# Niravaana/HIP-BVH-Construction

Hardware: AMD Instinct MI355X
Metric: bvh_build_throughput (higher is better)
Workload: dtype f32+u32

## Files before the change

### hip-bvh-construction_amd/csrc/api.hip

```cpp
#include <hip/hip_runtime.h>
#include <new>
#include <cstring>
#include <cstdlib>
#include "bvh_mi355x.h"
#include <mutex>
#include "common.hpp"
#include "kernels.hpp"

#include <vector>
#include <string>
#include <map>

using namespace bvh;

namespace bvh { thread_local KernelRecorder* g_recorder = nullptr; }

struct EventRecorder : KernelRecorder {
    struct Rec { const char* name; hipEvent_t ev; };
    std::vector<Rec> recs; size_t used = 0;
    std::string only;
    bool open = false;
    void mark(hipStream_t s, const char* name) override {
        if (!only.empty()) {
            const bool match = name && only == name;
// ... 11 lines not shown
struct bvh_ctx {
    int device = 0;
    hipStream_t stream = nullptr;
    bool own_stream = false;
    bool profiling = false;
    bool kernel_profiling = false;
    uint32_t sample_every = 1, build_counter = 0;
    EventRecorder recorder;
    uint32_t cap = 0;
    char* arena = nullptr;
    size_t arena_bytes = 0;
    void* tris = nullptr;
    uint32_t tris_cap = 0;
    bvh_aabb* boxes = nullptr;
    float* scene = nullptr;
    u32 *keys = nullptr, *skeys = nullptr, *svals = nullptr;
    SortScratch sort{};
    bvh2_node* nodes = nullptr;
    bvh_primref* leaves = nullptr;
    u64* slots = nullptr;
    u32* parent = nullptr;
    u32* flags = nullptr;
    HplocScratch hploc{};
    PlocScratch ploc{};
    u32* small = nullptr;
    u64* overlap_sums = nullptr;
    size_t lbvh_queue_capacity = 0;
    bool scratch_dirty = false;
    hipEvent_t ev[8] = {};
    int scene_slot = 0;
    bool scene_ready = false;
    uint32_t ploc_last_n = 0, ploc_last_iters = 0;
    u32* h_pinned = nullptr;
    u32* d_pinned = nullptr;
    float last_collapse_ms = 0.f;
    uint32_t collapse_last_n = 0, collapse_last_levels = 0;
    uint64_t collapse_last_key = 0;
    uint32_t collapse_last_len[COLLAPSE_MAX_BATCH] = {0};
    int collapse_len_batch = 0;
    int64_t options[4] = {0, 0, 0, 0};
    uint64_t tree_serial = 1, plan_serial = 0;
    uint32_t plan_n = 0, plan_root = 0;
    u32* subset_words = nullptr;
    uint32_t subset_cap = 0;
    bool subset_dirty = false;
    uint64_t map_serial = 0;
// ... 63 lines not shown
    __atomic_thread_fence(__ATOMIC_RELEASE);
}
static int read_back(bvh_ctx* c, const u32* d_a, u32 na, const u32* d_b, u32 nb, u32* pairs);

inline size_t align_up(size_t v, size_t a = 256) { return (v + a - 1) / a * a; }

struct Carver {
    char* base; size_t off = 0;
    template <typename T> T* take(size_t count) { T* p = base ? reinterpret_cast<T*>(base + off) : nullptr; off += align_up(count * sizeof(T)); return p; }
};

void carve(bvh_ctx* c, char* base, uint32_t cap, size_t* total) {
    Carver k{base};
    const size_t n = cap;
    c->boxes = k.take<bvh_aabb>(n);
    c->scene = k.take<float>(16);
    c->keys = reinterpret_cast<u32*>(k.take<u64>(n)); c->skeys = reinterpret_cast<u32*>(k.take<u64>(n)); c->svals = k.take<u32>(n);
    c->sort.pairs0 = k.take<uint4>(n); c->sort.pairs1 = k.take<uint4>(n);
    c->sort.hist = k.take<u32>(SORT_HIST_COPIES * SORT_HIST_STRIDE);
    c->sort.status = k.take<u32>(sort_status_bytes(cap) / sizeof(u32));
    c->sort.counters = k.take<u32>(SORT_MAX_PASSES);
    c->nodes = k.take<bvh2_node>(2 * n);
    c->leaves = k.take<bvh_primref>(n);
    c->slots = k.take<u64>(n);
    c->parent = k.take<u32>(2 * n);
    c->flags = k.take<u32>(n);
    c->hploc.recs = k.take<bvh2_node>(n);
    c->hploc.dep = k.take<u64>(n);
    c->hploc.queue_capacity = hploc_queue_capacity(cap);
    c->hploc.queue_pc = k.take<u32>(c->hploc.queue_capacity);
    c->hploc.queue_rng = k.take<u64>(c->hploc.queue_capacity);
// ... 11 lines not shown
}
inline u32* overflow_words(const bvh_ctx* c) { return c->small + 58; }
inline u64* total_word(const bvh_ctx* c) { return reinterpret_cast<u64*>(c->small + 60); }
inline u32* total_pairs(const bvh_ctx* c) { return c->h_pinned + 8; }

int ensure_capacity(bvh_ctx* c, uint32_t n) {
    if (n <= c->cap) return 0;
    HIP_TRY(hipStreamSynchronize(c->stream));
    if (c->arena) { HIP_TRY(hipFree(c->arena)); c->arena = nullptr; c->cap = 0; }
    size_t total = 0;
    carve(c, nullptr, n, &total);
    char* p = nullptr;
    HIP_TRY(hipMalloc(&p, total));
    c->arena = p; c->arena_bytes = total; c->cap = n;
    ++c->tree_serial;
    c->scene_ready = false; c->scene_slot = 0;
    carve(c, p, n, &total);
    HIP_TRY(hipMemsetAsync(c->hploc.dep, 0, (size_t)n * sizeof(u64), c->stream));
    HIP_TRY(hipMemsetAsync(c->flags, 0xFF, (size_t)n * sizeof(u32), c->stream));
    return 0;
}

int begin_emit(bvh_ctx* c) {
    if (c->scratch_dirty) {
        HIP_TRY(hipMemsetAsync(c->hploc.dep, 0, (size_t)c->cap * sizeof(u64), c->stream));
        HIP_TRY(hipMemsetAsync(c->flags, 0xFF, (size_t)c->cap * sizeof(u32), c->stream));
    }
    c->scratch_dirty = true;
    return 0;
}
int end_emit(bvh_ctx* c) {
// ... 64 lines not shown
            return 0;
        }
        first += batch; batch = 16;
    }
    return BVH_E_INTERNAL;
}

int stage_extents_valid(const bvh_build_input* in) {
    switch (in->tri_format) {
        case BVH_TRI_PADDED64: return in->d_tris ? 0 : BVH_E_INVALID_ARG;
        case BVH_TRI_PACKED36: return (in->d_tris && !((uintptr_t)in->d_tris & 15u)) ? 0 : BVH_E_INVALID_ARG;
        case BVH_TRI_INDEXED:  return (in->d_vertices && in->d_indices && in->n_vertices) ? 0 : BVH_E_INVALID_ARG;
        default: return BVH_E_INVALID_ARG;
    }
}
int stage_extents_fmt(hipStream_t s, const bvh_build_input* in, uint32_t n, void* d_boxes, void* d_scene, bool reset_scene = true, const PrepArgs* prep = nullptr) {
    const int v = stage_extents_valid(in); if (v) return v;
    switch (in->tri_format) {
        case BVH_TRI_PADDED64: launch_extents(s, in->d_tris, n, d_boxes, d_scene, reset_scene, prep); return 0;
        case BVH_TRI_PACKED36: launch_extents_packed(s, in->d_tris, n, d_boxes, d_scene, reset_scene, prep); return 0;
        case BVH_TRI_INDEXED:  launch_extents_indexed(s, in->d_vertices, in->d_indices, in->n_vertices, n, d_boxes, d_scene, reset_scene, prep); return 0;
        default: return BVH_E_INVALID_ARG;
    }
}

inline bool tree_valid(const bvh_result* tree) {
    const uint32_t n = tree->n_leaves;
    return !(n < 2 || tree->layout > 1u || !tree->d_nodes || (tree->layout == 1u && !tree->d_leaves) || tree->root >= n - 1);
}
int resolve_tris(const bvh_result* tree, const bvh_build_input* tris, bvh_build_input* in) {
    std::memset(in, 0, sizeof *in);
    if (tris) { if (stage_extents_valid(tris)) return BVH_E_INVALID_ARG; *in = *tris; }
    else { if (!tree->d_tris) return BVH_E_INVALID_ARG; in->tri_format = BVH_TRI_PADDED64; in->d_tris = tree->d_tris; }
    return 0;
}

struct Range { uintptr_t lo = 0, hi = 0;
    Range() = default;
// ... 192 lines not shown
int bvh_ctx_set_kernel_filter(bvh_ctx* c, const char* kernel_name) {
    if (!c) return BVH_E_INVALID_ARG;
    c->recorder.only = kernel_name ? kernel_name : ""; c->recorder.reset();
    return 0;
}
int bvh_ctx_set_kernel_sampling(bvh_ctx* c, uint32_t every) {
    if (!c || every == 0) return BVH_E_INVALID_ARG;
    c->sample_every = every; c->build_counter = 0; c->recorder.reset();
    return 0;
}
int bvh_ctx_synchronize(bvh_ctx* c) { if (!c) return BVH_E_INVALID_ARG; Bind b(c->device); return herr(hipStreamSynchronize(c->stream)); }

int bvh_stage_extents(bvh_ctx* c, const void* d_tris, uint32_t n, void* d_prim_aabbs, void* d_scene_extent) {
    if (!c || !d_tris || !d_prim_aabbs || !d_scene_extent || n == 0) return BVH_E_INVALID_ARG;
    Bind b(c->device);
    launch_extents(c->stream, d_tris, n, d_prim_aabbs, d_scene_extent);
    return herr(hipGetLastError());
}

int bvh_stage_morton(bvh_ctx* c, const void* d_prim_aabbs, uint32_t n, const void* d_scene_extent, uint32_t* d_keys, uint32_t* d_vals) {
    if (!c || !d_prim_aabbs || !d_scene_extent || !d_keys || n == 0) return BVH_E_INVALID_ARG;
    Bind b(c->device);
    launch_morton(c->stream, d_prim_aabbs, n, d_scene_extent, d_keys, d_vals, nullptr, 0, 0);
    return herr(hipGetLastError());
}

int bvh_sort_pairs(bvh_ctx* c, const uint32_t* d_keys_in, const uint32_t* d_vals_in, uint32_t n, uint32_t* d_keys_out,
                   uint32_t* d_vals_out, int start_bit, int end_bit) {
    if (!c || !d_keys_in || !d_keys_out || !d_vals_out || n == 0 || start_bit < 0 || end_bit > 32 || start_bit > end_bit) return BVH_E_INVALID_ARG;
    if (n >= (1u << 30)) return BVH_E_TOO_LARGE;
    Bind b(c->device);
// ... 23 lines not shown

int bvh_stage_morton_plan(bvh_ctx* c, const void* d_scene_extent, int total_bits, int32_t plan_out[10]) {
    if (!c || !d_scene_extent || !plan_out || total_bits < 3 || total_bits > 60) return BVH_E_INVALID_ARG;
    Bind b(c->device);
    int r = ensure_capacity(c, 2); if (r) return r;
    int* d = reinterpret_cast<int*>(c->small + 48);
    launch_morton_plan(c->stream, d_scene_extent, d, total_bits);
    HIP_TRY(hipGetLastError());
    HIP_TRY(hipMemcpyAsync(plan_out, d, 10 * sizeof(int32_t), hipMemcpyDeviceToHost, c->stream));
    return herr(hipStreamSynchronize(c->stream));
}

int bvh_stage_extents_ex(bvh_ctx* c, const bvh_build_input* in, uint32_t n, void* d_prim_aabbs, void* d_scene_extent) {
    if (!c || !in || !d_prim_aabbs || !d_scene_extent || n == 0) return BVH_E_INVALID_ARG;
    Bind b(c->device);
    int r = stage_extents_fmt(c->stream, in, n, d_prim_aabbs, d_scene_extent); if (r) return r;
    return herr(hipGetLastError());
}

int bvh_emit_lbvh_single(bvh_ctx* c, const void* d_prim_aabbs, const uint32_t* d_sorted_keys, const uint32_t* d_sorted_vals,
                         uint32_t n, void* d_nodes, uint32_t* root_out) {
    if (!c || !d_prim_aabbs || !d_sorted_keys || !d_sorted_vals || !d_nodes || n < 2) return BVH_E_INVALID_ARG;
    Bind b(c->device);
    int r = ensure_capacity(c, n); if (r) return r;
    ++c->tree_serial;
    r = begin_emit(c); if (r) return r;
    launch_lbvh_single(c->stream, d_prim_aabbs, d_sorted_keys, 32, d_sorted_vals, n, d_nodes, c->hploc.dep, c->small, c->ploc.list0, c->lbvh_queue_capacity, c->hploc.queue_count, false, (int)c->options[BVH_OPT_LBVH_SCHEDULER]);
    r = end_emit(c); if (r) return r;
    if (root_out) { r = read_back(c, c->small, 1, nullptr, 0, c->h_pinned); if (r) return r; *root_out = c->h_pinned[0]; }
    return 0;
}
// ... 38 lines not shown
#ifndef SORT_GATE_TOP
#define SORT_GATE_TOP 1
#endif
static int build_impl(bvh_ctx* c, bvh_algo algo, const bvh_build_input* in, uint32_t n, bvh_result* out, bvh_timings* tm, const void* d_in_boxes = nullptr) {
    const int key_bits = in->morton_bits == 60 ? 64 : 32;
    hipStream_t s = c->stream;
    Install install(c);
    const bool prof = c->profiling && install.sampled;
    uint32_t ploc_iters = 0;
    int r = 0;
    ++c->tree_serial;
    if (prof) HIP_TRY(hipEventRecord(c->ev[0], s));
    const int end_bit = key_bits == 64 ? 64 : (n >= SORT_WIDE_MIN_N && SORT_GATE_TOP != 0) ? 30 : 32;
    const int passes = sort_passes(0, end_bit);
    if (!d_in_boxes) { r = stage_extents_valid(in); if (r) return r; }
    float* const scene = c->scene + 8 * c->scene_slot;
    float* const scene_next = c->scene + 8 * (c->scene_slot ^ 1);
    PrepArgs prep;
    prep.hist = c->sort.hist; prep.hist_words = (u32)SORT_HIST_COPIES * SORT_HIST_STRIDE;
    prep.status = reinterpret_cast<uint4*>(c->sort.status); prep.status_vecs = (u32)(((size_t)passes * sort_tiles(n) * SORT_RADIX) / 4);
    prep.counters = c->sort.counters; prep.extra = c->hploc.queue_count; prep.extra_words = hploc_head_words();
    if (algo == BVH_PLOCPP) ploc_begin_prep(c->ploc, n, prep);
    const bool explicit_reset = !c->scene_ready;
    c->scene_ready = false;
    if (d_in_boxes) launch_extents_boxes(s, d_in_boxes, n, c->boxes, scene, explicit_reset, &prep);
    else { r = stage_extents_fmt(s, in, n, c->boxes, scene, explicit_reset, &prep); if (r) return r; }
    if (prof) HIP_TRY(hipEventRecord(c->ev[1], s));
    if (key_bits == 64) launch_morton64(s, c->boxes, n, scene, reinterpret_cast<u64*>(c->keys), 60, c->sort.hist, passes, scene_next);
    else launch_morton(s, c->boxes, n, scene, c->keys, nullptr, c->sort.hist, SORT_BITS, passes, scene_next);
    if (prof) HIP_TRY(hipEventRecord(c->ev[2], s));
    if (key_bits == 64) sort_pairs64(s, c->sort, reinterpret_cast<const u64*>(c->keys), nullptr, n, reinterpret_cast<u64*>(c->skeys), c->svals, 0, end_bit, true);
    else sort_pairs(s, c->sort, c->keys, nullptr, n, c->skeys, c->svals, 0, end_bit, true, end_bit == 30);
    if (prof) HIP_TRY(hipEventRecord(c->ev[3], s));
    out->d_leaves = nullptr; out->layout = 0; out->root = 0;
    r = begin_emit(c); if (r) return r;
    switch (algo) {
        case BVH_LBVH_SINGLEPASS: launch_lbvh_single(s, c->boxes, c->skeys, key_bits, c->svals, n, c->nodes, c->hploc.dep, c->small, c->ploc.list0, c->lbvh_queue_capacity, c->hploc.queue_count, true, (int)c->options[BVH_OPT_LBVH_SCHEDULER]); break;
        case BVH_LBVH_TWOPASS:    launch_lbvh_two(s, c->boxes, c->skeys, key_bits, c->svals, n, c->nodes, c->parent, c->flags, c->hploc.dep, c->small,
                                                  c->ploc.list0, c->lbvh_queue_capacity, c->hploc.queue_count, true, (int)c->options[BVH_OPT_LBVH_SCHEDULER]); break;
        case BVH_HPLOC:           c->hploc.leaf_tris = (LEAF_FROM_TRIS && !d_in_boxes && in->tri_format == BVH_TRI_PADDED64) ? in->d_tris : nullptr;
                                  emit_hploc(c, s, c->boxes, c->skeys, key_bits, c->svals, n, c->nodes, c->leaves, true);
                                  c->hploc.leaf_tris = nullptr;
                                  out->d_leaves = c->leaves; out->layout = 1; break;
        case BVH_PLOCPP:          r = run_ploc(c, n, c->nodes, c->leaves, c->boxes, c->svals, c->ploc, &ploc_iters); if (r) return r;
                                  out->d_leaves = c->leaves; out->layout = 1; break;
    }
    r = end_emit(c); if (r) return r;
    c->scene_ready = true; c->scene_slot ^= 1;
    install.mark();
    if (prof) HIP_TRY(hipEventRecord(c->ev[4], s));
    if (algo == BVH_LBVH_SINGLEPASS) {
        r = read_back(c, c->small, 1, nullptr, 0, c->h_pinned); if (r) return r;
        out->root = c->h_pinned[0];
        if (out->root >= 2u * n - 1u) return BVH_E_INTERNAL;
    }
    out->d_nodes = c->nodes; out->d_prim_aabbs = c->boxes; out->d_scene_extent = scene;
    out->d_sorted_keys = c->skeys; out->d_sorted_vals = c->svals;
    out->n_internal = n - 1; out->n_leaves = n; out->key_bits = (uint32_t)key_bits; out->reserved = 0;
    out->d_tris = d_in_boxes ? nullptr : in->tri_format == BVH_TRI_INDEXED ? in->d_vertices : in->d_tris; out->d_morton_keys = c->keys;
    if (tm) {
        std::memset(tm, 0, sizeof *tm);
        tm->bytes_algorithmic = algorithmic_bytes(algo, n);
        tm->ploc_iterations = ploc_iters;
// ... 45 lines not shown
    return build_impl(c, algo, &in, n, out, tm, d_boxes);
}

static int refit_check(const bvh_ctx* c, const bvh_result* io) {
    if (!c || !io) return BVH_E_INVALID_ARG;
    if (!tree_valid(io) || !io->d_prim_aabbs || !io->d_scene_extent) return BVH_E_INVALID_ARG;
    if (io->n_leaves > c->cap) return BVH_E_INVALID_ARG;
    return 0;
}
static int refit_impl(bvh_ctx* c, bvh_result* io, const bvh_build_input* in, bvh_timings* tm) {
    hipStream_t s = c->stream;
    const uint32_t n = io->n_leaves;
    Install install(c);
    const bool prof = c->profiling && install.sampled;
    if (prof) HIP_TRY(hipEventRecord(c->ev[0], s));
    int r = stage_extents_fmt(s, in, n, io->d_prim_aabbs, io->d_scene_extent, true, nullptr); if (r) return r;
    if (prof) HIP_TRY(hipEventRecord(c->ev[1], s));
    r = begin_emit(c); if (r) return r;
    const bool own = io->d_nodes == c->nodes;
    if (!own || c->plan_serial != c->tree_serial || c->plan_n != n || c->plan_root != io->root) {
        launch_refit_plan(s, io->d_nodes, n, io->root, c->parent);
        c->plan_serial = own ? c->tree_serial : 0; c->plan_n = n; c->plan_root = io->root;
    }
    launch_refit_climb(s, io->d_prim_aabbs, io->d_nodes, io->d_leaves, (int)io->layout, n, c->parent, c->flags);
    r = end_emit(c); if (r) { c->plan_serial = 0; return r; }
    install.mark();
    if (prof) HIP_TRY(hipEventRecord(c->ev[4], s));
    io->d_tris = in->tri_format == BVH_TRI_INDEXED ? in->d_vertices : in->d_tris;
    if (tm) {
        std::memset(tm, 0, sizeof *tm);
        tm->bytes_algorithmic = 200ull * n;
// ... 970 lines not shown
```

### hip-bvh-construction_amd/csrc/kernels.hpp

```cpp
#pragma once
#include <hip/hip_runtime.h>
#include <stdint.h>
#include "bvh/types.h"

namespace bvh {

struct KernelRecorder {
    virtual void mark(hipStream_t s, const char* name) = 0;
    virtual ~KernelRecorder() {}
};
extern thread_local KernelRecorder* g_recorder;
struct KernelScope {
    KernelScope(hipStream_t stream, const char* name) { if (g_recorder) g_recorder->mark(stream, name); }
};

constexpr int EM_BLOCK = 256;
struct PrepArgs { uint32_t* hist = nullptr; uint32_t hist_words = 0; uint4* status = nullptr; uint32_t status_vecs = 0; uint32_t* counters = nullptr;
                  uint32_t* extra = nullptr; uint32_t extra_words = 0;
                  uint4* ploc_status = nullptr; uint32_t ploc_status_vecs = 0; uint64_t* ploc_tail = nullptr; uint32_t ploc_tail_words = 0;
                  uint32_t* ploc_state = nullptr; uint32_t ploc_count = 0; };
#ifdef BVH_ABLATION
constexpr int SORT_COUNTER_CLEAR = 64;
#else
constexpr int SORT_COUNTER_CLEAR = 8;
#endif

void launch_extents(hipStream_t s, const void* d_tris, uint32_t n, void* d_boxes, void* d_scene, bool reset_scene = true, const PrepArgs* prep = nullptr);
void launch_extents_packed(hipStream_t s, const void* d_tris36, uint32_t n, void* d_boxes, void* d_scene, bool reset_scene = true, const PrepArgs* prep = nullptr);
void launch_extents_indexed(hipStream_t s, const void* d_vertices, const void* d_indices, uint32_t n_vertices, uint32_t n, void* d_boxes, void* d_scene, bool reset_scene = true, const PrepArgs* prep = nullptr);
void launch_extents_boxes(hipStream_t s, const void* d_in, uint32_t n, void* d_boxes, void* d_scene, bool reset_scene = true, const PrepArgs* prep = nullptr);
void launch_morton(hipStream_t s, const void* d_boxes, uint32_t n, const void* d_scene, uint32_t* d_keys, uint32_t* d_vals,
                   uint32_t* d_hist , int hist_bits, int passes, float* d_reset_next = nullptr );
void launch_morton64(hipStream_t s, const void* d_boxes, uint32_t n, const void* d_scene, uint64_t* d_keys, int total_bits,
                     uint32_t* d_hist , int passes, float* d_reset_next = nullptr);

void launch_morton_plan(hipStream_t s, const void* d_scene, int* d_out, int total_bits);

constexpr int SORT_BITS = 8;
constexpr int SORT_RADIX = 1 << SORT_BITS;
constexpr int SORT_BLOCK = 256;
#ifndef BVH_SORT_IPT
#define BVH_SORT_IPT 12
#endif
constexpr int SORT_IPT = BVH_SORT_IPT;
constexpr int SORT_TILE = SORT_BLOCK * SORT_IPT;
constexpr int SORT_IPT_WIDE = 20;
#ifndef BVH_SORT_WIDE_MIN_N
#define BVH_SORT_WIDE_MIN_N 1000000
#endif
// ... 198 lines not shown
```

### hip-bvh-construction_amd/csrc/stage_em.hip

```cpp
#include "common.hpp"
#include "kernels.hpp"
#include "morton.hpp"

namespace bvh {

__device__ __forceinline__ void atomic_min_f32(float* addr, float v) {
    if (__float_as_int(v) >= 0) atomicMin(reinterpret_cast<int*>(addr), __float_as_int(v));
    else atomicMax(reinterpret_cast<unsigned int*>(addr), __float_as_uint(v));
}
__device__ __forceinline__ void atomic_max_f32(float* addr, float v) {
    if (__float_as_int(v) >= 0) atomicMax(reinterpret_cast<int*>(addr), __float_as_int(v));
    else atomicMin(reinterpret_cast<unsigned int*>(addr), __float_as_uint(v));
}

__device__ __forceinline__ Box wave_reduce_box(Box b) {
#pragma unroll
    for (int m = 1; m < WAVE; m <<= 1) {
        b.lx = fminf(b.lx, __shfl_xor(b.lx, m)); b.ly = fminf(b.ly, __shfl_xor(b.ly, m)); b.lz = fminf(b.lz, __shfl_xor(b.lz, m));
        b.hx = fmaxf(b.hx, __shfl_xor(b.hx, m)); b.hy = fmaxf(b.hy, __shfl_xor(b.hy, m)); b.hz = fmaxf(b.hz, __shfl_xor(b.hz, m));
    }
    return b;
}

constexpr int EX_BLOCK = 1024;
__device__ __forceinline__ void block_reduce_scene(Box acc, float* __restrict__ scene) {
    acc = wave_reduce_box(acc);
    __shared__ float red[EX_BLOCK / WAVE][6];
    const int lane = threadIdx.x & (WAVE - 1), wave = threadIdx.x / WAVE, nw = blockDim.x / WAVE;
    if (lane == 0) { red[wave][0] = acc.lx; red[wave][1] = acc.ly; red[wave][2] = acc.lz; red[wave][3] = acc.hx; red[wave][4] = acc.hy; red[wave][5] = acc.hz; }
    __syncthreads();
    if (threadIdx.x < 6) {
        float v = red[0][threadIdx.x];
        for (int w = 1; w < nw; ++w) v = threadIdx.x < 3 ? fminf(v, red[w][threadIdx.x]) : fmaxf(v, red[w][threadIdx.x]);
        if (threadIdx.x < 3) atomic_min_f32(scene + threadIdx.x, v); else atomic_max_f32(scene + threadIdx.x, v);
    }
}

__device__ __forceinline__ void prep_slice(const PrepArgs& p) {
    const u32 t = blockIdx.x * blockDim.x + threadIdx.x, stride = gridDim.x * blockDim.x;
    for (u32 i = t; i < p.status_vecs; i += stride) p.status[i] = make_uint4(0u, 0u, 0u, 0u);
    for (u32 i = t; i < p.hist_words; i += stride) p.hist[i] = 0u;
    for (u32 i = t; i < p.extra_words; i += stride) p.extra[i] = 0u;
    if (p.counters && t < (u32)SORT_COUNTER_CLEAR) p.counters[t] = 0u;
    if (p.ploc_state) {
        for (u32 i = t; i < p.ploc_status_vecs; i += stride) p.ploc_status[i] = make_uint4(0u, 0u, 0u, 0u);
        if (t < p.ploc_tail_words) p.ploc_tail[t] = 0ull;
        if (t < (u32)PLOC_STATE_WORDS) p.ploc_state[t] = t == 0u ? p.ploc_count : 0u;
    }
}

__global__ __launch_bounds__(EX_BLOCK) void k_extents(const float4* __restrict__ tris, bvh_aabb* __restrict__ boxes,
                                                      float* __restrict__ scene, u32 n, PrepArgs prep) {
    prep_slice(prep);
    Box acc = box_empty();
    const u32 stride = gridDim.x * EX_BLOCK;
    for (u32 i = blockIdx.x * EX_BLOCK + threadIdx.x; i < n; i += stride) {
        const Box bx = stage_e_box_padded(tris, i);
        box_store(boxes + i, bx);
        acc = box_union(acc, bx);
    }
    block_reduce_scene(acc, scene);
}

__global__ __launch_bounds__(EM_BLOCK) void k_extents_packed(const float* __restrict__ tris, bvh_aabb* __restrict__ boxes,
                                                             float* __restrict__ scene, u32 n, PrepArgs prep) {
    prep_slice(prep);
    __shared__ float s_t[EM_BLOCK * 9];
    Box acc = box_empty();
    const u32 tiles = (n + EM_BLOCK - 1) / EM_BLOCK;
    for (u32 tile = blockIdx.x; tile < tiles; tile += gridDim.x) {
        const u32 base = tile * EM_BLOCK;
        const u32 cnt = (n - base) < (u32)EM_BLOCK ? (n - base) : (u32)EM_BLOCK;
        const float* src = tris + (size_t)base * 9;
        const u32 words = cnt * 9u, vecs = words / 4u;
        for (u32 v = threadIdx.x; v < vecs; v += EM_BLOCK) reinterpret_cast<float4*>(s_t)[v] = reinterpret_cast<const float4*>(src)[v];
        for (u32 k = vecs * 4u + threadIdx.x; k < words; k += EM_BLOCK) s_t[k] = src[k];
        __syncthreads();
        if (threadIdx.x < cnt) {
            const Box bx = stage_e_box9(s_t + threadIdx.x * 9);
            box_store(boxes + base + threadIdx.x, bx);
            acc = box_union(acc, bx);
        }
        __syncthreads();
    }
    block_reduce_scene(acc, scene);
}

__global__ __launch_bounds__(EX_BLOCK) void k_extents_indexed(const float* __restrict__ verts, const u32* __restrict__ idx, u32 n_verts,
                                                              bvh_aabb* __restrict__ boxes, float* __restrict__ scene, u32 n, PrepArgs prep) {
    prep_slice(prep);
    Box acc = box_empty();
    const u32 stride = gridDim.x * EX_BLOCK;
    for (u32 i = blockIdx.x * EX_BLOCK + threadIdx.x; i < n; i += stride) {
        const Box bx = stage_e_box_indexed(verts, idx, n_verts, i);
        box_store(boxes + i, bx);
        acc = box_union(acc, bx);
    }
    block_reduce_scene(acc, scene);
}

__global__ __launch_bounds__(EX_BLOCK) void k_extents_boxes(const bvh_aabb* in, bvh_aabb* boxes, float* __restrict__ scene, u32 n, PrepArgs prep) {
    prep_slice(prep);
    Box acc = box_empty();
    const u32 stride = gridDim.x * EX_BLOCK;
    for (u32 i = blockIdx.x * EX_BLOCK + threadIdx.x; i < n; i += stride) {
        const Box bx = box_load(in + i);
        box_store(boxes + i, bx);
        acc = box_union(acc, bx);
    }
    block_reduce_scene(acc, scene);
}

__global__ void k_reset_scene(float* scene) {
    if (threadIdx.x < 3) scene[threadIdx.x] = FMAX; else if (threadIdx.x < 6) scene[threadIdx.x] = -FMAX;
}


__device__ __forceinline__ u64 shl64(u64 v, u32 s) { return s >= 64u ? 0ull : v << s; }
__device__ __forceinline__ u64 shr64(u64 v, u32 s) { return s >= 64u ? 0ull : v >> s; }
__device__ __forceinline__ u64 spread2_64(u64 v) {
    v &= 0x00000000ffffffffull; v = (v ^ (v << 16)) & 0x0000ffff0000ffffull; v = (v ^ (v << 8)) & 0x00ff00ff00ff00ffull;
    v = (v ^ (v << 4)) & 0x0f0f0f0f0f0f0f0full; v = (v ^ (v << 2)) & 0x3333333333333333ull; v = (v ^ (v << 1)) & 0x5555555555555555ull; return v;
}
__device__ __forceinline__ u64 spread3_64(u64 x) {
    x &= 0x1fffffull; x = (x | (x << 32)) & 0x1f00000000ffffull; x = (x | (x << 16)) & 0x1f0000ff0000ffull;
    x = (x | (x << 8)) & 0x100f00f00f00f00full; x = (x | (x << 4)) & 0x10c30c30c30c30c3ull; x = (x | (x << 2)) & 0x1249249249249249ull; return x;
}
__device__ __forceinline__ u64 sat_f2u64(float f) {
    if (f != f) return 0ull;
// ... 22 lines not shown
        if (m.swap > 0) { code <<= 1; bx -= 1; code |= shr64(q0 & shl64(1ull, (u32)bx), (u32)bx); }
        code = shl64(code, (u32)(bx + by + bz));
        q0 &= shl64(1ull, (u32)bx) - 1ull;
        q1 &= shl64(1ull, (u32)by) - 1ull;
        if (m.swap > 0) { d0 = (u32)(by - bx); q0 = shl64(q0, d0); d1 = (u32)(by - bz); q2 = shl64(q2, d1); }
        else            { d0 = (u32)(bx - by); q1 = shl64(q1, d0); d1 = (u32)(bx - bz); q2 = shl64(q2, d1); }
    }
    if (bz == 0) code |= spread2_64(q0) * 2 + spread2_64(q1);
    else {
        const u64 X = spread3_64(q0), Y = spread3_64(q1), Z = spread3_64(q2);
        code |= shr64((m.swap > 0) ? (Y * 4 + X * 2 + Z) : (X * 4 + Y * 2 + Z), d0 + d1);
    }
    return code;
}

__global__ __launch_bounds__(EM_BLOCK) void k_morton64(const bvh_aabb* __restrict__ boxes, const float* __restrict__ scene,
                                                       u64* __restrict__ keys, u32 n, u32 total_bits, u32* __restrict__ hist, int passes, float* reset_next) {
    if (reset_next && blockIdx.x == 0 && threadIdx.x < 6) reset_next[threadIdx.x] = threadIdx.x < 3 ? FMAX : -FMAX;
    __shared__ MortonPlan s_plan; __shared__ float s_lo[3], s_ext[3];
    __shared__ u32 s_hist[8 * 256];
    __shared__ u32 s_pad[MORTON64_GROUP >= 3 ? 64 : 1];
    if (threadIdx.x == 0) make_plan(scene, s_plan, s_lo, s_ext, total_bits);
    for (int i = threadIdx.x; i < passes * 256; i += EM_BLOCK) s_hist[i] = 0;
    __syncthreads();
    const MortonPlan m = s_plan;
    const float lo[3] = { s_lo[0], s_lo[1], s_lo[2] }, ext[3] = { s_ext[0], s_ext[1], s_ext[2] };
    const u32 ntile = (n + EM_BLOCK - 1) / EM_BLOCK;
    for (u32 tile = blockIdx.x; tile < ntile; tile += gridDim.x) {
        const u32 i = (ntile - 1u - tile) * EM_BLOCK + threadIdx.x;
        if (i >= n) continue;
        const Box b = box_load(boxes + i);
        const float p[3] = { ((b.hx + b.lx) * 0.5f - lo[0]) / ext[0], ((b.hy + b.ly) * 0.5f - lo[1]) / ext[1], ((b.hz + b.lz) * 0.5f - lo[2]) / ext[2] };
        const u64 code = encode64(m, p[m.axis[0]], p[m.axis[1]], p[m.axis[2]]);
        keys[i] = code;
        hist_add_passes<MORTON64_GROUP>(s_hist, passes, 256, [&](int ps) { return (u32)(code >> (ps * 8)) & 255u; }, s_pad);
    }
    __syncthreads();
    u32* copy = hist + (blockIdx.x % SORT_HIST_COPIES) * SORT_HIST_STRIDE;
    for (int i = threadIdx.x; i < passes * 256; i += EM_BLOCK) { const u32 c = s_hist[i]; if (c) atomicAdd(&copy[i], c); }
}

template <int HIST_BITS>
__global__ __launch_bounds__(EM_BLOCK) void k_morton(const bvh_aabb* __restrict__ boxes, const float* __restrict__ scene,
                                                     u32* __restrict__ keys, u32* __restrict__ vals, u32 n,
                                                     u32* __restrict__ hist, int passes, float* reset_next) {
    if (reset_next && blockIdx.x == 0 && threadIdx.x < 6) reset_next[threadIdx.x] = threadIdx.x < 3 ? FMAX : -FMAX;
    __shared__ MortonPlan s_plan; __shared__ float s_lo[3], s_ext[3];
    constexpr int RADIX = HIST_BITS > 0 ? (1 << HIST_BITS) : 1;
    __shared__ u32 s_hist[HIST_BITS > 0 ? 4 * RADIX : 1];
    __shared__ u32 s_pad[MORTON_GROUP >= 3 ? 64 : 1];
    if (threadIdx.x == 0) make_plan(scene, s_plan, s_lo, s_ext);
    if (HIST_BITS > 0) for (int i = threadIdx.x; i < passes * RADIX; i += EM_BLOCK) s_hist[i] = 0;
    __syncthreads();
    const MortonPlan m = s_plan;
    const float lo[3] = { s_lo[0], s_lo[1], s_lo[2] }, ext[3] = { s_ext[0], s_ext[1], s_ext[2] };
    const u32 ntile = (n + EM_BLOCK - 1) / EM_BLOCK;
    for (u32 tile = blockIdx.x; tile < ntile; tile += gridDim.x) {
        const u32 i = (ntile - 1u - tile) * EM_BLOCK + threadIdx.x;
        if (i >= n) continue;
        const Box b = box_load(boxes + i);
        const float p[3] = { ((b.hx + b.lx) * 0.5f - lo[0]) / ext[0], ((b.hy + b.ly) * 0.5f - lo[1]) / ext[1], ((b.hz + b.lz) * 0.5f - lo[2]) / ext[2] };
        const u32 code = encode(m, p[m.axis[0]], p[m.axis[1]], p[m.axis[2]]);
// ... 14 lines not shown
            }
        }
    }
}

#ifndef EM_PPT
#define EM_PPT 4
#endif
#ifndef EX_PPT
#define EX_PPT 4
#endif
static inline int em_grid(u32 n) {
    const u32 blocks = (n + EM_PPT * EM_BLOCK - 1) / (EM_PPT * EM_BLOCK);
    return (int)(blocks < 2048u ? (blocks ? blocks : 1u) : 2048u);
}

static inline int ex_grid(u32 n) {
    const u32 blocks = (n + EX_PPT * EX_BLOCK - 1) / (EX_PPT * EX_BLOCK);
    return (int)(blocks < 512u ? (blocks ? blocks : 1u) : 512u);
}

void launch_extents(hipStream_t s, const void* d_tris, u32 n, void* d_boxes, void* d_scene, bool reset_scene, const PrepArgs* prep) {
    const PrepArgs pa = prep ? *prep : PrepArgs{};
    if (reset_scene) hipLaunchKernelGGL(k_reset_scene, dim3(1), dim3(64), 0, s, (float*)d_scene);
    KernelScope ks(s, "k_extents");
    hipLaunchKernelGGL(k_extents, dim3(ex_grid(n)), dim3(EX_BLOCK), 0, s, (const float4*)d_tris, (bvh_aabb*)d_boxes, (float*)d_scene, n, pa);
}

void launch_extents_packed(hipStream_t s, const void* d_tris36, u32 n, void* d_boxes, void* d_scene, bool reset_scene, const PrepArgs* prep) {
    const PrepArgs pa = prep ? *prep : PrepArgs{};
    if (reset_scene) hipLaunchKernelGGL(k_reset_scene, dim3(1), dim3(64), 0, s, (float*)d_scene);
    KernelScope ks(s, "k_extents_packed");
    hipLaunchKernelGGL(k_extents_packed, dim3(em_grid(n)), dim3(EM_BLOCK), 0, s, (const float*)d_tris36, (bvh_aabb*)d_boxes, (float*)d_scene, n, pa);
}
void launch_extents_indexed(hipStream_t s, const void* d_vertices, const void* d_indices, u32 n_vertices, u32 n, void* d_boxes, void* d_scene, bool reset_scene, const PrepArgs* prep) {
    const PrepArgs pa = prep ? *prep : PrepArgs{};
    if (reset_scene) hipLaunchKernelGGL(k_reset_scene, dim3(1), dim3(64), 0, s, (float*)d_scene);
    KernelScope ks(s, "k_extents_indexed");
    hipLaunchKernelGGL(k_extents_indexed, dim3(ex_grid(n)), dim3(EX_BLOCK), 0, s, (const float*)d_vertices, (const u32*)d_indices, n_vertices, (bvh_aabb*)d_boxes, (float*)d_scene, n, pa);
}

void launch_extents_boxes(hipStream_t s, const void* d_in, u32 n, void* d_boxes, void* d_scene, bool reset_scene, const PrepArgs* prep) {
    const PrepArgs pa = prep ? *prep : PrepArgs{};
    if (reset_scene) hipLaunchKernelGGL(k_reset_scene, dim3(1), dim3(64), 0, s, (float*)d_scene);
    KernelScope ks(s, "k_extents_boxes");
    hipLaunchKernelGGL(k_extents_boxes, dim3(ex_grid(n)), dim3(EX_BLOCK), 0, s, (const bvh_aabb*)d_in, (bvh_aabb*)d_boxes, (float*)d_scene, n, pa);
}
__global__ void k_morton_plan(const float* __restrict__ scene, int* __restrict__ out, u32 total_bits) {
    if (threadIdx.x != 0 || blockIdx.x != 0) return;
    MortonPlan m; float lo[3], ext[3];
    make_plan(scene, m, lo, ext, total_bits);
    for (int i = 0; i < 3; ++i) { out[i] = m.axis[i]; out[3 + i] = m.bits[i]; }
    out[6] = m.pre[0]; out[7] = m.pre[1]; out[8] = m.pre_sum; out[9] = m.swap;
}
void launch_morton_plan(hipStream_t s, const void* d_scene, int* d_out, int total_bits) {
    hipLaunchKernelGGL(k_morton_plan, dim3(1), dim3(64), 0, s, (const float*)d_scene, d_out, (u32)total_bits);
}

void launch_morton(hipStream_t s, const void* d_boxes, u32 n, const void* d_scene, u32* d_keys, u32* d_vals,
                   u32* d_hist, int hist_bits, int passes, float* d_reset_next) {
    const dim3 g(em_grid(n)), b(EM_BLOCK);
    KernelScope ks(s, "k_morton");
    if (d_hist && hist_bits == 8)       hipLaunchKernelGGL(k_morton<8>,  g, b, 0, s, (const bvh_aabb*)d_boxes, (const float*)d_scene, d_keys, d_vals, n, d_hist, passes, d_reset_next);
    else                                hipLaunchKernelGGL(k_morton<0>,  g, b, 0, s, (const bvh_aabb*)d_boxes, (const float*)d_scene, d_keys, d_vals, n, (u32*)nullptr, 0, d_reset_next);
}

void launch_morton64(hipStream_t s, const void* d_boxes, u32 n, const void* d_scene, uint64_t* d_keys, int total_bits, u32* d_hist, int passes, float* d_reset_next) {
    KernelScope ks(s, "k_morton64");
    hipLaunchKernelGGL(k_morton64, dim3(em_grid(n)), dim3(EM_BLOCK), 0, s, (const bvh_aabb*)d_boxes, (const float*)d_scene, d_keys, n, (u32)total_bits,
                       d_hist, d_hist ? passes : 0, d_reset_next);
}

void warm_stage_em() { hipFuncAttributes a; (void)hipFuncGetAttributes(&a, reinterpret_cast<const void*>(&k_reset_scene)); }

}
```

Baseline: 8535.

## Replace atomic scene-extent reduction with per-block partials folded in morton kernel

```diff
diff --git a/hip-bvh-construction_amd/csrc/api.hip b/hip-bvh-construction_amd/csrc/api.hip
--- a/hip-bvh-construction_amd/csrc/api.hip
+++ b/hip-bvh-construction_amd/csrc/api.hip
@@ -49,6 +49,7 @@
     uint32_t tris_cap = 0;
     bvh_aabb* boxes = nullptr;
     float* scene = nullptr;
+    float* partials = nullptr;
     u32 *keys = nullptr, *skeys = nullptr, *svals = nullptr;
     SortScratch sort{};
     bvh2_node* nodes = nullptr;
@@ -63,8 +64,6 @@
     size_t lbvh_queue_capacity = 0;
     bool scratch_dirty = false;
     hipEvent_t ev[8] = {};
-    int scene_slot = 0;
-    bool scene_ready = false;
     uint32_t ploc_last_n = 0, ploc_last_iters = 0;
     u32* h_pinned = nullptr;
     u32* d_pinned = nullptr;
@@ -158,7 +157,8 @@
     Carver k{base};
     const size_t n = cap;
     c->boxes = k.take<bvh_aabb>(n);
-    c->scene = k.take<float>(16);
+    c->scene = k.take<float>(8);
+    c->partials = k.take<float>(6 * (size_t)EX_MAX_PARTIALS);
     c->keys = reinterpret_cast<u32*>(k.take<u64>(n)); c->skeys = reinterpret_cast<u32*>(k.take<u64>(n)); c->svals = k.take<u32>(n);
     c->sort.pairs0 = k.take<uint4>(n); c->sort.pairs1 = k.take<uint4>(n);
     c->sort.hist = k.take<u32>(SORT_HIST_COPIES * SORT_HIST_STRIDE);
@@ -200,7 +200,6 @@
     HIP_TRY(hipMalloc(&p, total));
     c->arena = p; c->arena_bytes = total; c->cap = n;
     ++c->tree_serial;
-    c->scene_ready = false; c->scene_slot = 0;
     carve(c, p, n, &total);
     HIP_TRY(hipMemsetAsync(c->hploc.dep, 0, (size_t)n * sizeof(u64), c->stream));
     HIP_TRY(hipMemsetAsync(c->flags, 0xFF, (size_t)n * sizeof(u32), c->stream));
@@ -295,14 +294,17 @@
         default: return BVH_E_INVALID_ARG;
     }
 }
-int stage_extents_fmt(hipStream_t s, const bvh_build_input* in, uint32_t n, void* d_boxes, void* d_scene, bool reset_scene = true, const PrepArgs* prep = nullptr) {
+int stage_extents_fmt(hipStream_t s, const bvh_build_input* in, uint32_t n, void* d_boxes, float* d_partials, void* d_scene, const PrepArgs* prep = nullptr, uint32_t* n_partials = nullptr) {
     const int v = stage_extents_valid(in); if (v) return v;
+    uint32_t count = 0;
     switch (in->tri_format) {
-        case BVH_TRI_PADDED64: launch_extents(s, in->d_tris, n, d_boxes, d_scene, reset_scene, prep); return 0;
-        case BVH_TRI_PACKED36: launch_extents_packed(s, in->d_tris, n, d_boxes, d_scene, reset_scene, prep); return 0;
-        case BVH_TRI_INDEXED:  launch_extents_indexed(s, in->d_vertices, in->d_indices, in->n_vertices, n, d_boxes, d_scene, reset_scene, prep); return 0;
+        case BVH_TRI_PADDED64: count = launch_extents(s, in->d_tris, n, d_boxes, d_partials, d_scene, prep); break;
+        case BVH_TRI_PACKED36: count = launch_extents_packed(s, in->d_tris, n, d_boxes, d_partials, d_scene, prep); break;
+        case BVH_TRI_INDEXED:  count = launch_extents_indexed(s, in->d_vertices, in->d_indices, in->n_vertices, n, d_boxes, d_partials, d_scene, prep); break;
         default: return BVH_E_INVALID_ARG;
     }
+    if (n_partials) *n_partials = count;
+    return 0;
 }
 
 inline bool tree_valid(const bvh_result* tree) {
@@ -525,7 +527,8 @@
 int bvh_stage_extents(bvh_ctx* c, const void* d_tris, uint32_t n, void* d_prim_aabbs, void* d_scene_extent) {
     if (!c || !d_tris || !d_prim_aabbs || !d_scene_extent || n == 0) return BVH_E_INVALID_ARG;
     Bind b(c->device);
-    launch_extents(c->stream, d_tris, n, d_prim_aabbs, d_scene_extent);
+    int r = ensure_capacity(c, 2); if (r) return r;
+    launch_extents(c->stream, d_tris, n, d_prim_aabbs, c->partials, d_scene_extent);
     return herr(hipGetLastError());
 }
 
@@ -579,7 +582,9 @@
 int bvh_stage_extents_ex(bvh_ctx* c, const bvh_build_input* in, uint32_t n, void* d_prim_aabbs, void* d_scene_extent) {
     if (!c || !in || !d_prim_aabbs || !d_scene_extent || n == 0) return BVH_E_INVALID_ARG;
     Bind b(c->device);
-    int r = stage_extents_fmt(c->stream, in, n, d_prim_aabbs, d_scene_extent); if (r) return r;
+    int r = stage_extents_valid(in); if (r) return r;
+    r = ensure_capacity(c, 2); if (r) return r;
+    r = stage_extents_fmt(c->stream, in, n, d_prim_aabbs, c->partials, d_scene_extent); if (r) return r;
     return herr(hipGetLastError());
 }
 
@@ -648,20 +653,18 @@
     const int end_bit = key_bits == 64 ? 64 : (n >= SORT_WIDE_MIN_N && SORT_GATE_TOP != 0) ? 30 : 32;
     const int passes = sort_passes(0, end_bit);
     if (!d_in_boxes) { r = stage_extents_valid(in); if (r) return r; }
-    float* const scene = c->scene + 8 * c->scene_slot;
-    float* const scene_next = c->scene + 8 * (c->scene_slot ^ 1);
+    float* const scene = c->scene;
+    uint32_t n_partials = 0;
     PrepArgs prep;
     prep.hist = c->sort.hist; prep.hist_words = (u32)SORT_HIST_COPIES * SORT_HIST_STRIDE;
     prep.status = reinterpret_cast<uint4*>(c->sort.status); prep.status_vecs = (u32)(((size_t)passes * sort_tiles(n) * SORT_RADIX) / 4);
     prep.counters = c->sort.counters; prep.extra = c->hploc.queue_count; prep.extra_words = hploc_head_words();
     if (algo == BVH_PLOCPP) ploc_begin_prep(c->ploc, n, prep);
-    const bool explicit_reset = !c->scene_ready;
-    c->scene_ready = false;
-    if (d_in_boxes) launch_extents_boxes(s, d_in_boxes, n, c->boxes, scene, explicit_reset, &prep);
-    else { r = stage_extents_fmt(s, in, n, c->boxes, scene, explicit_reset, &prep); if (r) return r; }
+    if (d_in_boxes) n_partials = launch_extents_boxes(s, d_in_boxes, n, c->boxes, c->partials, nullptr, &prep);
+    else { r = stage_extents_fmt(s, in, n, c->boxes, c->partials, nullptr, &prep, &n_partials); if (r) return r; }
     if (prof) HIP_TRY(hipEventRecord(c->ev[1], s));
-    if (key_bits == 64) launch_morton64(s, c->boxes, n, scene, reinterpret_cast<u64*>(c->keys), 60, c->sort.hist, passes, scene_next);
-    else launch_morton(s, c->boxes, n, scene, c->keys, nullptr, c->sort.hist, SORT_BITS, passes, scene_next);
+    if (key_bits == 64) launch_morton64(s, c->boxes, n, scene, reinterpret_cast<u64*>(c->keys), 60, c->sort.hist, passes, c->partials, n_partials, scene);
+    else launch_morton(s, c->boxes, n, scene, c->keys, nullptr, c->sort.hist, SORT_BITS, passes, c->partials, n_partials, scene);
     if (prof) HIP_TRY(hipEventRecord(c->ev[2], s));
     if (key_bits == 64) sort_pairs64(s, c->sort, reinterpret_cast<const u64*>(c->keys), nullptr, n, reinterpret_cast<u64*>(c->skeys), c->svals, 0, end_bit, true);
     else sort_pairs(s, c->sort, c->keys, nullptr, n, c->skeys, c->svals, 0, end_bit, true, end_bit == 30);
@@ -680,7 +683,6 @@
                                   out->d_leaves = c->leaves; out->layout = 1; break;
     }
     r = end_emit(c); if (r) return r;
-    c->scene_ready = true; c->scene_slot ^= 1;
     install.mark();
     if (prof) HIP_TRY(hipEventRecord(c->ev[4], s));
     if (algo == BVH_LBVH_SINGLEPASS) {
@@ -756,7 +758,7 @@
     Install install(c);
     const bool prof = c->profiling && install.sampled;
     if (prof) HIP_TRY(hipEventRecord(c->ev[0], s));
-    int r = stage_extents_fmt(s, in, n, io->d_prim_aabbs, io->d_scene_extent, true, nullptr); if (r) return r;
+    int r = stage_extents_fmt(s, in, n, io->d_prim_aabbs, c->partials, io->d_scene_extent); if (r) return r;
     if (prof) HIP_TRY(hipEventRecord(c->ev[1], s));
     r = begin_emit(c); if (r) return r;
     const bool own = io->d_nodes == c->nodes;
diff --git a/hip-bvh-construction_amd/csrc/kernels.hpp b/hip-bvh-construction_amd/csrc/kernels.hpp
--- a/hip-bvh-construction_amd/csrc/kernels.hpp
+++ b/hip-bvh-construction_amd/csrc/kernels.hpp
@@ -25,14 +25,15 @@
 constexpr int SORT_COUNTER_CLEAR = 8;
 #endif
 
-void launch_extents(hipStream_t s, const void* d_tris, uint32_t n, void* d_boxes, void* d_scene, bool reset_scene = true, const PrepArgs* prep = nullptr);
-void launch_extents_packed(hipStream_t s, const void* d_tris36, uint32_t n, void* d_boxes, void* d_scene, bool reset_scene = true, const PrepArgs* prep = nullptr);
-void launch_extents_indexed(hipStream_t s, const void* d_vertices, const void* d_indices, uint32_t n_vertices, uint32_t n, void* d_boxes, void* d_scene, bool reset_scene = true, const PrepArgs* prep = nullptr);
-void launch_extents_boxes(hipStream_t s, const void* d_in, uint32_t n, void* d_boxes, void* d_scene, bool reset_scene = true, const PrepArgs* prep = nullptr);
+constexpr uint32_t EX_MAX_PARTIALS = 2048;
+uint32_t launch_extents(hipStream_t s, const void* d_tris, uint32_t n, void* d_boxes, float* d_partials, void* d_scene, const PrepArgs* prep = nullptr);
+uint32_t launch_extents_packed(hipStream_t s, const void* d_tris36, uint32_t n, void* d_boxes, float* d_partials, void* d_scene, const PrepArgs* prep = nullptr);
+uint32_t launch_extents_indexed(hipStream_t s, const void* d_vertices, const void* d_indices, uint32_t n_vertices, uint32_t n, void* d_boxes, float* d_partials, void* d_scene, const PrepArgs* prep = nullptr);
+uint32_t launch_extents_boxes(hipStream_t s, const void* d_in, uint32_t n, void* d_boxes, float* d_partials, void* d_scene, const PrepArgs* prep = nullptr);
 void launch_morton(hipStream_t s, const void* d_boxes, uint32_t n, const void* d_scene, uint32_t* d_keys, uint32_t* d_vals,
-                   uint32_t* d_hist , int hist_bits, int passes, float* d_reset_next = nullptr );
+                   uint32_t* d_hist , int hist_bits, int passes, const float* d_partials = nullptr, uint32_t n_partials = 0, float* d_scene_out = nullptr);
 void launch_morton64(hipStream_t s, const void* d_boxes, uint32_t n, const void* d_scene, uint64_t* d_keys, int total_bits,
-                     uint32_t* d_hist , int passes, float* d_reset_next = nullptr);
+                     uint32_t* d_hist , int passes, const float* d_partials = nullptr, uint32_t n_partials = 0, float* d_scene_out = nullptr);
 
 void launch_morton_plan(hipStream_t s, const void* d_scene, int* d_out, int total_bits);
 
diff --git a/hip-bvh-construction_amd/csrc/stage_em.hip b/hip-bvh-construction_amd/csrc/stage_em.hip
--- a/hip-bvh-construction_amd/csrc/stage_em.hip
+++ b/hip-bvh-construction_amd/csrc/stage_em.hip
@@ -4,15 +4,6 @@
 
 namespace bvh {
 
-__device__ __forceinline__ void atomic_min_f32(float* addr, float v) {
-    if (__float_as_int(v) >= 0) atomicMin(reinterpret_cast<int*>(addr), __float_as_int(v));
-    else atomicMax(reinterpret_cast<unsigned int*>(addr), __float_as_uint(v));
-}
-__device__ __forceinline__ void atomic_max_f32(float* addr, float v) {
-    if (__float_as_int(v) >= 0) atomicMax(reinterpret_cast<int*>(addr), __float_as_int(v));
-    else atomicMin(reinterpret_cast<unsigned int*>(addr), __float_as_uint(v));
-}
-
 __device__ __forceinline__ Box wave_reduce_box(Box b) {
 #pragma unroll
     for (int m = 1; m < WAVE; m <<= 1) {
@@ -22,8 +13,9 @@
     return b;
 }
 
-constexpr int EX_BLOCK = 1024;
-__device__ __forceinline__ void block_reduce_scene(Box acc, float* __restrict__ scene) {
+constexpr int EX_BLOCK = 512;
+static_assert(EX_BLOCK % WAVE == 0 && EX_BLOCK >= EM_BLOCK && EX_BLOCK <= 1024, "stage-E workgroup: whole waves, EM_BLOCK (k_extents_packed) .. 1024 threads");
+__device__ __forceinline__ void block_reduce_scene(Box acc, float* __restrict__ partials) {
     acc = wave_reduce_box(acc);
     __shared__ float red[EX_BLOCK / WAVE][6];
     const int lane = threadIdx.x & (WAVE - 1), wave = threadIdx.x / WAVE, nw = blockDim.x / WAVE;
@@ -32,7 +24,41 @@
     if (threadIdx.x < 6) {
         float v = red[0][threadIdx.x];
         for (int w = 1; w < nw; ++w) v = threadIdx.x < 3 ? fminf(v, red[w][threadIdx.x]) : fmaxf(v, red[w][threadIdx.x]);
-        if (threadIdx.x < 3) atomic_min_f32(scene + threadIdx.x, v); else atomic_max_f32(scene + threadIdx.x, v);
+        partials[threadIdx.x * EX_MAX_PARTIALS + blockIdx.x] = v;
+    }
+}
+
+constexpr int FOLD_BLOCK = EM_BLOCK;
+__device__ __forceinline__ int fold_key(float v) { const int b = __float_as_int(v); return b >= 0 ? b : b ^ 0x7fffffff; }
+__device__ __forceinline__ float fold_val(int k) { return __int_as_float(k >= 0 ? k : k ^ 0x7fffffff); }
+__device__ __forceinline__ void fold_partials(const float* __restrict__ partials, u32 count, float* out ) {
+    __shared__ int s_fold[FOLD_BLOCK / WAVE][6];
+    int k[6] = { fold_key(FMAX), fold_key(FMAX), fold_key(FMAX), fold_key(-FMAX), fold_key(-FMAX), fold_key(-FMAX) };
+    for (u32 i = 2u * threadIdx.x; i < count; i += 2u * FOLD_BLOCK) {
+        const bool two = i + 1u < count;
+        float2 v[6];
+#pragma unroll
+        for (int j = 0; j < 6; ++j) v[j] = *reinterpret_cast<const float2*>(partials + j * EX_MAX_PARTIALS + i);
+#pragma unroll
+        for (int j = 0; j < 6; ++j) {
+            const int a = fold_key(v[j].x), b = two ? fold_key(v[j].y) : a;
+            k[j] = j < 3 ? min(k[j], min(a, b)) : max(k[j], max(a, b));
+        }
+    }
+#pragma unroll
+    for (int m = 1; m < WAVE; m <<= 1) {
+#pragma unroll
+        for (int j = 0; j < 3; ++j) { k[j] = min(k[j], __shfl_xor(k[j], m)); k[3 + j] = max(k[3 + j], __shfl_xor(k[3 + j], m)); }
+    }
+    const int lane = threadIdx.x & (WAVE - 1), wave = threadIdx.x / WAVE;
+    if (lane == 0) { for (int j = 0; j < 6; ++j) s_fold[wave][j] = k[j]; }
+    __syncthreads();
+    if (threadIdx.x == 0) {
+        for (int j = 0; j < 6; ++j) {
+            int v = s_fold[0][j];
+            for (int w = 1; w < FOLD_BLOCK / WAVE; ++w) v = j < 3 ? min(v, s_fold[w][j]) : max(v, s_fold[w][j]);
+            out[j] = fold_val(v);
+        }
     }
 }
 
@@ -50,7 +76,7 @@
 }
 
 __global__ __launch_bounds__(EX_BLOCK) void k_extents(const float4* __restrict__ tris, bvh_aabb* __restrict__ boxes,
-                                                      float* __restrict__ scene, u32 n, PrepArgs prep) {
+                                                      float* __restrict__ partials, u32 n, PrepArgs prep) {
     prep_slice(prep);
     Box acc = box_empty();
     const u32 stride = gridDim.x * EX_BLOCK;
@@ -59,11 +85,11 @@
         box_store(boxes + i, bx);
         acc = box_union(acc, bx);
     }
-    block_reduce_scene(acc, scene);
+    block_reduce_scene(acc, partials);
 }
 
 __global__ __launch_bounds__(EM_BLOCK) void k_extents_packed(const float* __restrict__ tris, bvh_aabb* __restrict__ boxes,
-                                                             float* __restrict__ scene, u32 n, PrepArgs prep) {
+                                                             float* __restrict__ partials, u32 n, PrepArgs prep) {
     prep_slice(prep);
     __shared__ float s_t[EM_BLOCK * 9];
     Box acc = box_empty();
@@ -83,11 +109,11 @@
         }
         __syncthreads();
     }
-    block_reduce_scene(acc, scene);
+    block_reduce_scene(acc, partials);
 }
 
 __global__ __launch_bounds__(EX_BLOCK) void k_extents_indexed(const float* __restrict__ verts, const u32* __restrict__ idx, u32 n_verts,
-                                                              bvh_aabb* __restrict__ boxes, float* __restrict__ scene, u32 n, PrepArgs prep) {
+                                                              bvh_aabb* __restrict__ boxes, float* __restrict__ partials, u32 n, PrepArgs prep) {
     prep_slice(prep);
     Box acc = box_empty();
     const u32 stride = gridDim.x * EX_BLOCK;
@@ -96,10 +122,10 @@
         box_store(boxes + i, bx);
         acc = box_union(acc, bx);
     }
-    block_reduce_scene(acc, scene);
-}
-
-__global__ __launch_bounds__(EX_BLOCK) void k_extents_boxes(const bvh_aabb* in, bvh_aabb* boxes, float* __restrict__ scene, u32 n, PrepArgs prep) {
+    block_reduce_scene(acc, partials);
+}
+
+__global__ __launch_bounds__(EX_BLOCK) void k_extents_boxes(const bvh_aabb* in, bvh_aabb* boxes, float* __restrict__ partials, u32 n, PrepArgs prep) {
     prep_slice(prep);
     Box acc = box_empty();
     const u32 stride = gridDim.x * EX_BLOCK;
@@ -108,11 +134,13 @@
         box_store(boxes + i, bx);
         acc = box_union(acc, bx);
     }
-    block_reduce_scene(acc, scene);
-}
-
-__global__ void k_reset_scene(float* scene) {
-    if (threadIdx.x < 3) scene[threadIdx.x] = FMAX; else if (threadIdx.x < 6) scene[threadIdx.x] = -FMAX;
+    block_reduce_scene(acc, partials);
+}
+
+__global__ __launch_bounds__(FOLD_BLOCK) void k_fold_scene(const float* __restrict__ partials, u32 count, float* __restrict__ scene) {
+    __shared__ float s_scene[6];
+    fold_partials(partials, count, s_scene);
+    if (threadIdx.x == 0) { for (int j = 0; j < 6; ++j) scene[j] = s_scene[j]; }
 }
 
 
@@ -165,10 +193,19 @@
     return code;
 }
 
-__global__ __launch_bounds__(EM_BLOCK) void k_morton64(const bvh_aabb* __restrict__ boxes, const float* __restrict__ scene,
-                                                       u64* __restrict__ keys, u32 n, u32 total_bits, u32* __restrict__ hist, int passes, float* reset_next) {
-    if (reset_next && blockIdx.x == 0 && threadIdx.x < 6) reset_next[threadIdx.x] = threadIdx.x < 3 ? FMAX : -FMAX;
-    __shared__ MortonPlan s_plan; __shared__ float s_lo[3], s_ext[3];
+__device__ __forceinline__ const float* morton_scene(const float* __restrict__ scene, const float* __restrict__ partials, u32 n_partials,
+                                                     float* __restrict__ scene_out, float* s_scene) {
+    if (n_partials == 0u) return scene;
+    fold_partials(partials, n_partials, s_scene);
+    if (blockIdx.x == 0 && threadIdx.x == 0) { for (int j = 0; j < 6; ++j) scene_out[j] = s_scene[j]; }
+    return s_scene;
+}
+
+__global__ __launch_bounds__(EM_BLOCK) void k_morton64(const bvh_aabb* __restrict__ boxes, const float* scene,
+                                                       u64* __restrict__ keys, u32 n, u32 total_bits, u32* __restrict__ hist, int passes,
+                                                       const float* __restrict__ partials, u32 n_partials, float* __restrict__ scene_out) {
+    __shared__ MortonPlan s_plan; __shared__ float s_lo[3], s_ext[3], s_scene[6];
+    scene = morton_scene(scene, partials, n_partials, scene_out, s_scene);
     __shared__ u32 s_hist[8 * 256];
     __shared__ u32 s_pad[MORTON64_GROUP >= 3 ? 64 : 1];
     if (threadIdx.x == 0) make_plan(scene, s_plan, s_lo, s_ext, total_bits);
@@ -192,11 +229,12 @@
 }
 
 template <int HIST_BITS>
-__global__ __launch_bounds__(EM_BLOCK) void k_morton(const bvh_aabb* __restrict__ boxes, const float* __restrict__ scene,
+__global__ __launch_bounds__(EM_BLOCK) void k_morton(const bvh_aabb* __restrict__ boxes, const float* scene,
                                                      u32* __restrict__ keys, u32* __restrict__ vals, u32 n,
-                                                     u32* __restrict__ hist, int passes, float* reset_next) {
-    if (reset_next && blockIdx.x == 0 && threadIdx.x < 6) reset_next[threadIdx.x] = threadIdx.x < 3 ? FMAX : -FMAX;
-    __shared__ MortonPlan s_plan; __shared__ float s_lo[3], s_ext[3];
+                                                     u32* __restrict__ hist, int passes,
+                                                     const float* __restrict__ partials, u32 n_partials, float* __restrict__ scene_out) {
+    __shared__ MortonPlan s_plan; __shared__ float s_lo[3], s_ext[3], s_scene[6];
+    scene = morton_scene(scene, partials, n_partials, scene_out, s_scene);
     constexpr int RADIX = HIST_BITS > 0 ? (1 << HIST_BITS) : 1;
     __shared__ u32 s_hist[HIST_BITS > 0 ? 4 * RADIX : 1];
     __shared__ u32 s_pad[MORTON_GROUP >= 3 ? 64 : 1];
@@ -241,37 +279,49 @@
     const u32 blocks = (n + EM_PPT * EM_BLOCK - 1) / (EM_PPT * EM_BLOCK);
     return (int)(blocks < 2048u ? (blocks ? blocks : 1u) : 2048u);
 }
-
+static_assert(EX_MAX_PARTIALS >= 2048, "k_extents_packed runs on em_grid");
+
+constexpr int EX_MAX_GRID = 1024;
+static_assert(EX_MAX_GRID <= EX_MAX_PARTIALS, "one partial box per workgroup");
 static inline int ex_grid(u32 n) {
     const u32 blocks = (n + EX_PPT * EX_BLOCK - 1) / (EX_PPT * EX_BLOCK);
-    return (int)(blocks < 512u ? (blocks ? blocks : 1u) : 512u);
-}
-
-void launch_extents(hipStream_t s, const void* d_tris, u32 n, void* d_boxes, void* d_scene, bool reset_scene, const PrepArgs* prep) {
+    return (int)(blocks < (u32)EX_MAX_GRID ? (blocks ? blocks : 1u) : (u32)EX_MAX_GRID);
+}
+
+static inline u32 finish_extents(hipStream_t s, int grid, const float* d_partials, void* d_scene) {
+    if (d_scene) hipLaunchKernelGGL(k_fold_scene, dim3(1), dim3(FOLD_BLOCK), 0, s, d_partials, (u32)grid, (float*)d_scene);
+    return (u32)grid;
+}
+
+u32 launch_extents(hipStream_t s, const void* d_tris, u32 n, void* d_boxes, float* d_partials, void* d_scene, const PrepArgs* prep) {
     const PrepArgs pa = prep ? *prep : PrepArgs{};
-    if (reset_scene) hipLaunchKernelGGL(k_reset_scene, dim3(1), dim3(64), 0, s, (float*)d_scene);
-    KernelScope ks(s, "k_extents");
-    hipLaunchKernelGGL(k_extents, dim3(ex_grid(n)), dim3(EX_BLOCK), 0, s, (const float4*)d_tris, (bvh_aabb*)d_boxes, (float*)d_scene, n, pa);
-}
-
-void launch_extents_packed(hipStream_t s, const void* d_tris36, u32 n, void* d_boxes, void* d_scene, bool reset_scene, const PrepArgs* prep) {
+    const int grid = ex_grid(n);
+    { KernelScope ks(s, "k_extents");
+      hipLaunchKernelGGL(k_extents, dim3(grid), dim3(EX_BLOCK), 0, s, (const float4*)d_tris, (bvh_aabb*)d_boxes, d_partials, n, pa); }
+    return finish_extents(s, grid, d_partials, d_scene);
+}
+
+u32 launch_extents_packed(hipStream_t s, const void* d_tris36, u32 n, void* d_boxes, float* d_partials, void* d_scene, const PrepArgs* prep) {
     const PrepArgs pa = prep ? *prep : PrepArgs{};
-    if (reset_scene) hipLaunchKernelGGL(k_reset_scene, dim3(1), dim3(64), 0, s, (float*)d_scene);
-    KernelScope ks(s, "k_extents_packed");
-    hipLaunchKernelGGL(k_extents_packed, dim3(em_grid(n)), dim3(EM_BLOCK), 0, s, (const float*)d_tris36, (bvh_aabb*)d_boxes, (float*)d_scene, n, pa);
-}
-void launch_extents_indexed(hipStream_t s, const void* d_vertices, const void* d_indices, u32 n_vertices, u32 n, void* d_boxes, void* d_scene, bool reset_scene, const PrepArgs* prep) {
+    const int grid = em_grid(n);
+    { KernelScope ks(s, "k_extents_packed");
+      hipLaunchKernelGGL(k_extents_packed, dim3(grid), dim3(EM_BLOCK), 0, s, (const float*)d_tris36, (bvh_aabb*)d_boxes, d_partials, n, pa); }
+    return finish_extents(s, grid, d_partials, d_scene);
+}
+u32 launch_extents_indexed(hipStream_t s, const void* d_vertices, const void* d_indices, u32 n_vertices, u32 n, void* d_boxes, float* d_partials, void* d_scene, const PrepArgs* prep) {
     const PrepArgs pa = prep ? *prep : PrepArgs{};
-    if (reset_scene) hipLaunchKernelGGL(k_reset_scene, dim3(1), dim3(64), 0, s, (float*)d_scene);
-    KernelScope ks(s, "k_extents_indexed");
-    hipLaunchKernelGGL(k_extents_indexed, dim3(ex_grid(n)), dim3(EX_BLOCK), 0, s, (const float*)d_vertices, (const u32*)d_indices, n_vertices, (bvh_aabb*)d_boxes, (float*)d_scene, n, pa);
-}
-
-void launch_extents_boxes(hipStream_t s, const void* d_in, u32 n, void* d_boxes, void* d_scene, bool reset_scene, const PrepArgs* prep) {
+    const int grid = ex_grid(n);
+    { KernelScope ks(s, "k_extents_indexed");
+      hipLaunchKernelGGL(k_extents_indexed, dim3(grid), dim3(EX_BLOCK), 0, s, (const float*)d_vertices, (const u32*)d_indices, n_vertices, (bvh_aabb*)d_boxes, d_partials, n, pa); }
+    return finish_extents(s, grid, d_partials, d_scene);
+}
+
+u32 launch_extents_boxes(hipStream_t s, const void* d_in, u32 n, void* d_boxes, float* d_partials, void* d_scene, const PrepArgs* prep) {
     const PrepArgs pa = prep ? *prep : PrepArgs{};
-    if (reset_scene) hipLaunchKernelGGL(k_reset_scene, dim3(1), dim3(64), 0, s, (float*)d_scene);
-    KernelScope ks(s, "k_extents_boxes");
-    hipLaunchKernelGGL(k_extents_boxes, dim3(ex_grid(n)), dim3(EX_BLOCK), 0, s, (const bvh_aabb*)d_in, (bvh_aabb*)d_boxes, (float*)d_scene, n, pa);
+    const int grid = ex_grid(n);
+    { KernelScope ks(s, "k_extents_boxes");
+      hipLaunchKernelGGL(k_extents_boxes, dim3(grid), dim3(EX_BLOCK), 0, s, (const bvh_aabb*)d_in, (bvh_aabb*)d_boxes, d_partials, n, pa); }
+    return finish_extents(s, grid, d_partials, d_scene);
 }
 __global__ void k_morton_plan(const float* __restrict__ scene, int* __restrict__ out, u32 total_bits) {
     if (threadIdx.x != 0 || blockIdx.x != 0) return;
@@ -285,19 +335,20 @@
 }
 
 void launch_morton(hipStream_t s, const void* d_boxes, u32 n, const void* d_scene, u32* d_keys, u32* d_vals,
-                   u32* d_hist, int hist_bits, int passes, float* d_reset_next) {
+                   u32* d_hist, int hist_bits, int passes, const float* d_partials, u32 n_partials, float* d_scene_out) {
     const dim3 g(em_grid(n)), b(EM_BLOCK);
     KernelScope ks(s, "k_morton");
-    if (d_hist && hist_bits == 8)       hipLaunchKernelGGL(k_morton<8>,  g, b, 0, s, (const bvh_aabb*)d_boxes, (const float*)d_scene, d_keys, d_vals, n, d_hist, passes, d_reset_next);
-    else                                hipLaunchKernelGGL(k_morton<0>,  g, b, 0, s, (const bvh_aabb*)d_boxes, (const float*)d_scene, d_keys, d_vals, n, (u32*)nullptr, 0, d_reset_next);
-}
-
-void launch_morton64(hipStream_t s, const void* d_boxes, u32 n, const void* d_scene, uint64_t* d_keys, int total_bits, u32* d_hist, int passes, float* d_reset_next) {
+    if (d_hist && hist_bits == 8)       hipLaunchKernelGGL(k_morton<8>,  g, b, 0, s, (const bvh_aabb*)d_boxes, (const float*)d_scene, d_keys, d_vals, n, d_hist, passes, d_partials, n_partials, d_scene_out);
+    else                                hipLaunchKernelGGL(k_morton<0>,  g, b, 0, s, (const bvh_aabb*)d_boxes, (const float*)d_scene, d_keys, d_vals, n, (u32*)nullptr, 0, d_partials, n_partials, d_scene_out);
+}
+
+void launch_morton64(hipStream_t s, const void* d_boxes, u32 n, const void* d_scene, uint64_t* d_keys, int total_bits, u32* d_hist, int passes,
+                     const float* d_partials, u32 n_partials, float* d_scene_out) {
     KernelScope ks(s, "k_morton64");
     hipLaunchKernelGGL(k_morton64, dim3(em_grid(n)), dim3(EM_BLOCK), 0, s, (const bvh_aabb*)d_boxes, (const float*)d_scene, d_keys, n, (u32)total_bits,
-                       d_hist, d_hist ? passes : 0, d_reset_next);
-}
-
-void warm_stage_em() { hipFuncAttributes a; (void)hipFuncGetAttributes(&a, reinterpret_cast<const void*>(&k_reset_scene)); }
-
-}
+                       d_hist, d_hist ? passes : 0, d_partials, n_partials, d_scene_out);
+}
+
+void warm_stage_em() { hipFuncAttributes a; (void)hipFuncGetAttributes(&a, reinterpret_cast<const void*>(&k_fold_scene)); }
+
+}
```

Result: no change. 8534 (-0.0%).
